# enoche/MMRec

Hardware: AMD Instinct MI355X
Metric: GCN-layer edges/sec (3-layer user-item CSR SpMM, d=64, fp32) (higher is better)
Workload: dtype f32

## Files before the change

### include/mmrec_hip.h

```cpp
#ifndef MMREC_HIP_H
#define MMREC_HIP_H

#include <stddef.h>
#include <stdint.h>

#ifdef __cplusplus
extern "C" {
#endif

#define MMREC_ABI_VERSION 16
#define MMREC_EMB_DIM 64

#define MMREC_ERR_BAD_ARG 10001
#define MMREC_ERR_UNSUPPORTED 10002

typedef void* mmrec_stream_t;

int mmrec_abi_version(void);
const char* mmrec_error_string(int err);

#ifndef MMREC_SPMM_CHUNK
#define MMREC_SPMM_CHUNK 512
#endif
#define MMREC_SPMM_LONG_ROW_DEFAULT 32
// ... 24 lines not shown
                             const float* Z, const float* acc_in, float* acc_out, int32_t n_rows, int32_t d, float alpha,
                             float beta, float acc_scale, int32_t long_row_threshold, const int32_t* long_rows,
                             const int32_t* long_chunk_ptr, int32_t n_long, int32_t n_chunks, float* partials,
                             int32_t* long_tickets, const int32_t* sched_row, const int32_t* sched_span,
                             const int32_t* sched_col, const float* sched_val, int32_t n_short, mmrec_stream_t stream);
int mmrec_spmm_csr_sched_f32_layergcn(const int32_t* rowptr, const int32_t* colidx, const float* vals, const float* X,
                                      float* Y, const float* ego, float* scaled, float* w, const float* acc_in,
                                      float* acc_out, int32_t n_rows, int32_t d, int32_t long_row_threshold,
                                      const int32_t* long_rows, const int32_t* long_chunk_ptr, int32_t n_long,
                                      int32_t n_chunks, float* partials, int32_t* long_tickets, const int32_t* sched_row,
                                      const int32_t* sched_span, const int32_t* sched_col, const float* sched_val,
                                      int32_t n_short, mmrec_stream_t stream);
int mmrec_spmm_row_keys(const int32_t* rowptr, const int32_t* colidx, const int32_t* col_degree, int32_t n_rows,
                        int32_t long_row_threshold, int32_t key_deg_max, int32_t* key, int32_t* key_degree,
                        mmrec_stream_t stream);

int mmrec_spmm_csr_masked_f32(const int32_t* rowptr, const int32_t* colidx, const float* vals, const float* X, float* Y,
                              const float* Z, const float* acc_in, float* acc_out, int32_t n_rows, int32_t d, float alpha,
                              float beta, float acc_scale, int32_t long_row_threshold, const int32_t* long_rows,
                              const int32_t* long_chunk_ptr, int32_t n_long, int32_t n_chunks, float* partials,
                              int32_t* long_tickets, const uint32_t* keep_bits, float val_scale, mmrec_stream_t stream);
int mmrec_edge_keep_bits(const uint8_t* keep, int64_t n_edges, const int64_t* perm_a, uint32_t* bits_a,
                         const int64_t* perm_b, uint32_t* bits_b, mmrec_stream_t stream);
int mmrec_spmm_plan_count(const int32_t* rowptr_host, int32_t n_rows, int32_t long_row_threshold,
                          int32_t* n_long, int32_t* n_chunks);
int mmrec_spmm_plan_fill(const int32_t* rowptr_host, int32_t n_rows, int32_t long_row_threshold,
                         int32_t* long_rows, int32_t* long_chunk_ptr);

int mmrec_cos_scale_fwd_f32(const float* E, const float* Ego, float* Out, float* w, float* acc,
                            int32_t n_rows, int32_t d, mmrec_stream_t stream);
int mmrec_cos_scale_bwd_f32(const float* dOut, const float* E, const float* Ego, const float* w,
                            float* dE, float* dEgo_accum, int32_t n_rows, int32_t d,
                            mmrec_stream_t stream);

#define MMREC_BPR_LOGSIG 0
#define MMREC_BPR_GAMMA 1

size_t mmrec_bpr_workspace_bytes(int32_t batch);
int mmrec_bpr_fwd_f32(const float* U, const float* P, const float* N, const int64_t* users,
                      const int64_t* pos, const int64_t* neg, int32_t batch, int32_t d,
                      int32_t variant, float scale, float* loss_out, float* coef, void* workspace,
                      mmrec_stream_t stream);
int mmrec_bpr_bwd_f32(const float* U, const float* P, const float* N, const int64_t* users,
                      const int64_t* pos, const int64_t* neg, int32_t batch, int32_t d,
                      const float* coef, const float* grad_scalar, float scale, float* dU, float* dP,
                      float* dN, mmrec_stream_t stream);
// ... 224 lines not shown
```

### mmrec_amd/_lib.py

```python
from __future__ import annotations

import ctypes
import os
from ctypes import c_char_p, c_float, c_int32, c_int64, c_size_t, c_uint64, c_void_p

import torch

_PKG = os.path.dirname(os.path.abspath(__file__))
LIB_PATH = os.environ.get("MMREC_HIP_LIB") or os.path.join(_PKG, "lib", "libmmrec_hip.so")
ABI_VERSION = 16

_P = c_void_p

SIGNATURES = {
    "mmrec_abi_version": (c_int32, []),
    "mmrec_error_string": (c_char_p, [c_int32]),
    "mmrec_spmm_csr_f32": (c_int32, [_P, _P, _P, _P, _P, _P, _P, _P, c_int32, c_int32, c_float,
                                     c_float, c_float, c_int32, _P, _P, c_int32, c_int32, _P, _P, _P]),
    "mmrec_spmm_csr_f32_layergcn": (c_int32, [_P, _P, _P, _P, _P, _P, _P, _P, _P, _P, c_int32, c_int32, c_int32,
                                              _P, _P, c_int32, c_int32, _P, _P, _P]),
    "mmrec_spmm_csr_sched_f32": (c_int32, [_P, _P, _P, _P, _P, _P, _P, _P, c_int32, c_int32, c_float,
                                           c_float, c_float, c_int32, _P, _P, c_int32, c_int32, _P, _P,
                                           _P, _P, _P, _P, c_int32, _P]),
    "mmrec_spmm_csr_sched_f32_layergcn": (c_int32, [_P, _P, _P, _P, _P, _P, _P, _P, _P, _P, c_int32, c_int32, c_int32,
                                                    _P, _P, c_int32, c_int32, _P, _P, _P, _P, _P, _P, c_int32, _P]),
    "mmrec_spmm_csr_masked_f32": (c_int32, [_P, _P, _P, _P, _P, _P, _P, _P, c_int32, c_int32, c_float,
                                            c_float, c_float, c_int32, _P, _P, c_int32, c_int32, _P, _P, _P, c_float, _P]),
    "mmrec_edge_keep_bits": (c_int32, [_P, c_int64, _P, _P, _P, _P, _P]),
    "mmrec_spmm_row_keys": (c_int32, [_P, _P, _P, c_int32, c_int32, c_int32, _P, _P, _P]),
    "mmrec_spmm_plan_count": (c_int32, [_P, c_int32, c_int32, _P, _P]),
    "mmrec_spmm_plan_fill": (c_int32, [_P, c_int32, c_int32, _P, _P]),
    "mmrec_cos_scale_fwd_f32": (c_int32, [_P, _P, _P, _P, _P, c_int32, c_int32, _P]),
    "mmrec_cos_scale_bwd_f32": (c_int32, [_P, _P, _P, _P, _P, _P, c_int32, c_int32, _P]),
    "mmrec_bpr_workspace_bytes": (c_size_t, [c_int32]),
    "mmrec_bpr_fwd_f32": (c_int32, [_P, _P, _P, _P, _P, _P, c_int32, c_int32, c_int32, c_float, _P,
                                    _P, _P, _P]),
    "mmrec_spmm_rows_f32": (c_int32, [_P, _P, _P, _P, _P, c_int32, _P, c_int32, c_int32, c_int32, _P, _P]),
    "mmrec_spmm_rows_any_f32": (c_int32, [_P, _P, _P, _P, _P, c_int32, _P, c_int32, c_int32, c_int32, c_int32, _P, _P]),
    "mmrec_spmm_push_rows_f32": (c_int32, [_P, _P, _P, _P, c_float, _P, c_int32, c_int32, _P, _P, _P]),
    "mmrec_bpr_dots_f32": (c_int32, [_P, _P, _P, _P, _P, _P, c_int32, c_int32, _P, _P]),
    "mmrec_bpr_loss_from_dots_f32": (c_int32, [_P, c_int32, c_int32, c_float, _P, _P, _P, _P]),
    "mmrec_bpr_bwd_f32": (c_int32, [_P, _P, _P, _P, _P, _P, c_int32, c_int32, _P, _P, c_float, _P, _P,
                                    _P, _P]),
    "mmrec_gather_sqnorm_fwd_f32": (c_int32, [_P, _P, c_int32, c_int32, _P, _P, _P]),
    "mmrec_gather_scale_add_bwd_f32": (c_int32, [_P, _P, c_int32, c_int32, _P, _P, _P]),
    "mmrec_infonce_workspace_bytes": (c_size_t, [c_int32]),
    "mmrec_infonce_fwd_f32": (c_int32, [_P, _P, _P, c_int32, c_int32, c_float, _P, _P, _P]),
    "mmrec_infonce_bwd_f32": (c_int32, [_P, c_int32, c_int32, c_float, _P, _P, _P, _P, _P]),
    "mmrec_linear_workspace_bytes": (c_size_t, [c_int32, c_int32, c_int32]),
    "mmrec_linear_fwd_f32": (c_int32, [_P, _P, _P, _P, c_int32, c_int32, c_int32, _P, _P]),
# ... 118 lines not shown
```

### mmrec_amd/csrc/spmm.hip

```cpp
#include "common.h"
#include "spmm_narrow.h"

#ifndef MMREC_SPMM_RPG
#define MMREC_SPMM_RPG(n_rows) ((n_rows) <= (1 << 18) ? 1 : 4)
#endif

namespace {

__device__ __forceinline__ void st_coherent(float4* p, float4 v) {
    unsigned long long* q = reinterpret_cast<unsigned long long*>(p);
    const unsigned long long lo = ((unsigned long long)__float_as_uint(v.y) << 32) | __float_as_uint(v.x);
    const unsigned long long hi = ((unsigned long long)__float_as_uint(v.w) << 32) | __float_as_uint(v.z);
    __hip_atomic_store(q, lo, __ATOMIC_RELAXED, __HIP_MEMORY_SCOPE_AGENT);
    __hip_atomic_store(q + 1, hi, __ATOMIC_RELAXED, __HIP_MEMORY_SCOPE_AGENT);
}
__device__ __forceinline__ float4 ld_coherent(const float4* p) {
    unsigned long long* q = reinterpret_cast<unsigned long long*>(const_cast<float4*>(p));
    const unsigned long long lo = __hip_atomic_load(q, __ATOMIC_RELAXED, __HIP_MEMORY_SCOPE_AGENT);
    const unsigned long long hi = __hip_atomic_load(q + 1, __ATOMIC_RELAXED, __HIP_MEMORY_SCOPE_AGENT);
    return make_float4(__uint_as_float((unsigned)lo), __uint_as_float((unsigned)(lo >> 32)),
                       __uint_as_float((unsigned)hi), __uint_as_float((unsigned)(hi >> 32)));
}

struct RowEpilogue {
    const float* Z;
    float* Y;
    const float* acc_in;
    float* acc_out;
    float alpha, beta, acc_scale;
    const float* ego;
    float* scaled;
    float* w_out;
};

struct RowSchedule {
    const int32_t* row;
    const int2* span;
    const int32_t* col;
    const float* val;
    int n_short;
};

template <int DCH, bool LG>
__device__ __forceinline__ void store_row(const RowEpilogue& ep, int row, int lane16, const float4 (&sum)[DCH]) {
    if (DCH == 1 && LG) {
        const size_t off = (size_t)row * 16 + lane16;
        const float4 y = f4_scale(ep.alpha, sum[0]);
        const float4 g = reinterpret_cast<const float4*>(ep.ego)[off];
        const float dot = row16_sum(f4_dot(y, g));
        const float ne = fmaxf(sqrtf(row16_sum(f4_dot(y, y))), 1e-8f);
        const float ng = fmaxf(sqrtf(row16_sum(f4_dot(g, g))), 1e-8f);
        const float w = dot / (ne * ng);
        const float4 o = f4_scale(w, y);
        if (ep.Y) reinterpret_cast<float4*>(ep.Y)[off] = y;
        reinterpret_cast<float4*>(ep.scaled)[off] = o;
        if (lane16 == 0) ep.w_out[row] = w;
        if (ep.acc_out)
            reinterpret_cast<float4*>(ep.acc_out)[off] =
                ep.acc_in ? f4_add(reinterpret_cast<const float4*>(ep.acc_in)[off], o) : o;
        return;
    }
#pragma unroll
    for (int ch = 0; ch < DCH; ++ch) {
        const size_t off = (size_t)row * (16 * DCH) + ch * 16 + lane16;
        float4 y = f4_scale(ep.alpha, sum[ch]);
        if (ep.Z) y = f4_fma(ep.beta, reinterpret_cast<const float4*>(ep.Z)[off], y);
        if (ep.Y) reinterpret_cast<float4*>(ep.Y)[off] = y;
// ... 19 lines not shown
            v = vals[k];
        }
        const int cnt = min(16, e - base);
        for (int j0 = 0; j0 < cnt; j0 += NB) {
            float4 x[NB][DCH];
            float vv[NB];
#pragma unroll
            for (int u = 0; u < NB; ++u) {
                const int j = j0 + u;
                const int cj = __shfl(c, j, 16);
                vv[u] = __shfl(v, j, 16);
#pragma unroll
                for (int ch = 0; ch < DCH; ++ch)
                    x[u][ch] = (j < cnt) ? X4[(size_t)cj * (16 * DCH) + ch * 16 + lane16] : f4_zero();
            }
#pragma unroll
            for (int u = 0; u < NB; ++u)
#pragma unroll
                for (int ch = 0; ch < DCH; ++ch) acc[ch] = f4_fma(vv[u], x[u][ch], acc[ch]);
        }
    }
}

template <int DCH, bool COHERENT, bool LG>
__device__ __forceinline__ void reduce_long_row(const float* __restrict__ partials, int c0, int c1, int row,
                                                const RowEpilogue& ep, float4 (*red)[16 * DCH]) {
    const int lane16 = threadIdx.x & 15, g = threadIdx.x >> 4;
#pragma unroll
    for (int ch = 0; ch < DCH; ++ch) {
        float4 t = f4_zero();
        for (int c = c0 + g; c < c1; c += 16) {
            const float4* src = reinterpret_cast<const float4*>(partials) + (size_t)c * (16 * DCH) + ch * 16 + lane16;
            t = f4_add(t, COHERENT ? ld_coherent(src) : *src);
        }
        red[g][ch * 16 + lane16] = t;
    }
    __syncthreads();
    if (g == 0) {
        float4 r[DCH];
#pragma unroll
        for (int ch = 0; ch < DCH; ++ch) {
            r[ch] = red[0][ch * 16 + lane16];
#pragma unroll
            for (int k = 1; k < 16; ++k) r[ch] = f4_add(r[ch], red[k][ch * 16 + lane16]);
        }
        store_row<DCH, LG>(ep, row, lane16, r);
    }
}

template <int DCH, bool LG, bool SCHED>
__global__ __launch_bounds__(256) void spmm_rows_kernel(
    const int32_t* __restrict__ rowptr, const int32_t* __restrict__ colidx,
    const float* __restrict__ vals, const float* __restrict__ X, RowEpilogue ep, int n_rows,
    int long_t, int rows_per_group, const int32_t* __restrict__ long_rows,
    const int32_t* __restrict__ long_chunk_ptr, int n_long, int n_chunks,
    float* __restrict__ partials, int32_t* __restrict__ tickets, RowSchedule sched) {
    __shared__ float4 red[16][16 * DCH];
    __shared__ int s_last;
    const int lane16 = threadIdx.x & 15;
    const int g = threadIdx.x >> 4;
    const float4* X4 = reinterpret_cast<const float4*>(X);
    if ((int)blockIdx.x < n_chunks) {
        const int chunk = blockIdx.x;
        int lo = 0, hi = n_long;
        while (hi - lo > 1) {
            const int mid = (lo + hi) >> 1;
            if (long_chunk_ptr[mid] <= chunk) lo = mid; else hi = mid;
        }
        const int row = long_rows[lo];
        const int cs = rowptr[row] + (chunk - long_chunk_ptr[lo]) * MMREC_SPMM_CHUNK;
        const int ce = min(cs + MMREC_SPMM_CHUNK, rowptr[row + 1]);
        float4 acc[DCH];
#pragma unroll
        for (int ch = 0; ch < DCH; ++ch) acc[ch] = f4_zero();
        for (int base = cs + g * 16; base < ce; base += 256)
            gather_span<DCH>(colidx, vals, X4, base, min(base + 16, ce), lane16, acc);
#pragma unroll
        for (int ch = 0; ch < DCH; ++ch) red[g][ch * 16 + lane16] = acc[ch];
        __syncthreads();
        if (g == 0) {
            float4 t[DCH];
#pragma unroll
            for (int ch = 0; ch < DCH; ++ch) {
                t[ch] = red[0][ch * 16 + lane16];
#pragma unroll
                for (int i = 1; i < 16; ++i) t[ch] = f4_add(t[ch], red[i][ch * 16 + lane16]);
            }
            if (long_chunk_ptr[lo + 1] - long_chunk_ptr[lo] == 1) {
                store_row<DCH, LG>(ep, row, lane16, t);
            } else {
#pragma unroll
                for (int ch = 0; ch < DCH; ++ch) {
                    float4* dst = reinterpret_cast<float4*>(partials) + (size_t)chunk * (16 * DCH) + ch * 16 + lane16;
                    if (tickets) st_coherent(dst, t[ch]); else *dst = t[ch];
                }
            }
        }
        const int c0 = long_chunk_ptr[lo], c1 = long_chunk_ptr[lo + 1];
        if (!tickets || c1 - c0 == 1) return;
        if (threadIdx.x < 64) {
            __atomic_signal_fence(__ATOMIC_SEQ_CST);
            __builtin_amdgcn_s_waitcnt(0);
            __atomic_signal_fence(__ATOMIC_SEQ_CST);
            __builtin_amdgcn_fence(__ATOMIC_RELEASE, "workgroup");
            if (threadIdx.x == 0)
                s_last = __hip_atomic_fetch_add(tickets + lo, 1, __ATOMIC_RELAXED, __HIP_MEMORY_SCOPE_AGENT) == c1 - c0 - 1;
        }
        __syncthreads();
        if (!s_last) return;
        __builtin_amdgcn_fence(__ATOMIC_ACQUIRE, "workgroup");
        reduce_long_row<DCH, true, LG>(partials, c0, c1, row, ep, red);
        if (threadIdx.x == 0) __hip_atomic_store(tickets + lo, 0, __ATOMIC_RELAXED, __HIP_MEMORY_SCOPE_AGENT);
        return;
    }
    if (SCHED) {
        const int slot0 = ((int)blockIdx.x - n_chunks) * 16 * rows_per_group + g;
#pragma unroll 1
        for (int i = 0; i < rows_per_group; ++i) {
            const int slot = slot0 + i * 16;
            if (slot >= sched.n_short) break;
            const int row = sched.row[slot];
            const int2 se = sched.span[slot];
            float4 acc[DCH];
#pragma unroll
            for (int ch = 0; ch < DCH; ++ch) acc[ch] = f4_zero();
            gather_span<DCH>(sched.col, sched.val, X4, se.x, se.y, lane16, acc);
            store_row<DCH, LG>(ep, row, lane16, acc);
        }
        return;
    }
    const int row0 = ((int)blockIdx.x - n_chunks) * 16 * rows_per_group + g;
#pragma unroll 1
    for (int i = 0; i < rows_per_group; ++i) {
        const int row = row0 + i * 16;
        if (row >= n_rows) break;
        const int s = rowptr[row], e = rowptr[row + 1];
        if (e - s > long_t) continue;
        float4 acc[DCH];
#pragma unroll
        for (int ch = 0; ch < DCH; ++ch) acc[ch] = f4_zero();
        gather_span<DCH>(colidx, vals, X4, s, e, lane16, acc);
        store_row<DCH, LG>(ep, row, lane16, acc);
    }
}

template <int DCH, bool LG>
__global__ __launch_bounds__(256) void spmm_long_reduce_kernel(
    const int32_t* __restrict__ long_rows, const int32_t* __restrict__ long_chunk_ptr, int n_long,
    const float* __restrict__ partials, RowEpilogue ep) {
    __shared__ float4 red[16][16 * DCH];
    const int i = blockIdx.x;
    const int c0 = long_chunk_ptr[i], c1 = long_chunk_ptr[i + 1];
    if (c1 - c0 <= 1) return;
    reduce_long_row<DCH, false, LG>(partials, c0, c1, long_rows[i], ep, red);
}

template <int DCH, bool LG = false, bool SCHED = false>
void launch_spmm(hipStream_t s, int blocks, int nch, const int32_t* rowptr, const int32_t* colidx,
                 const float* vals, const float* X, const RowEpilogue& ep, int n_rows, int long_t,
                 int rows_per_group, const int32_t* long_rows, const int32_t* long_chunk_ptr, int n_long,
                 float* partials, int32_t* tickets, const RowSchedule& sched = RowSchedule{}) {
    if (blocks + nch > 0)
        hipLaunchKernelGGL((spmm_rows_kernel<DCH, LG, SCHED>), dim3(blocks + nch), dim3(256), 0, s, rowptr, colidx, vals, X,
                           ep, n_rows, long_t, rows_per_group, long_rows, long_chunk_ptr, n_long, nch, partials, tickets,
                           sched);
    if (!tickets && n_long > 0 && nch > n_long)
        hipLaunchKernelGGL((spmm_long_reduce_kernel<DCH, LG>), dim3(n_long), dim3(256), 0, s, long_rows,
                           long_chunk_ptr, n_long, partials, ep);
}

template <int DCH>
__device__ __forceinline__ void gather_span_masked(const int32_t* __restrict__ colidx, const float* __restrict__ vals,
                                                   const uint32_t* __restrict__ keep_bits, float val_scale,
                                                   const float4* __restrict__ X4, int s, int e, int lane16,
                                                   float4 (&acc)[DCH]) {
    constexpr int NB = DCH == 1 ? 8 : (DCH <= 2 ? 4 : (DCH <= 4 ? 2 : 1));
    const int gshift = threadIdx.x & 48;
    for (int base = s; base < e; base += 16) {
        const int k = base + lane16;
        int c = 0;
        float v = 0.f;
        bool kept = false;
        if (k < e) {
            kept = (keep_bits[k >> 5] >> (k & 31)) & 1u;
            c = colidx[k];
            v = vals[k] * val_scale;
        }
        unsigned m = (unsigned)(__ballot(kept) >> gshift) & 0xffffu;
        while (m) {
            float4 x[NB][DCH];
            float vv[NB];
#pragma unroll
            for (int u = 0; u < NB; ++u) {
                const bool on = m != 0;
                const int j = on ? __ffs(m) - 1 : 0;
                m &= m - 1;
                const int cj = __shfl(c, j, 16);
                const float vj = __shfl(v, j, 16);
                vv[u] = on ? vj : 0.f;
#pragma unroll
                for (int ch = 0; ch < DCH; ++ch)
                    x[u][ch] = on ? X4[(size_t)cj * (16 * DCH) + ch * 16 + lane16] : f4_zero();
            }
#pragma unroll
            for (int u = 0; u < NB; ++u)
#pragma unroll
                for (int ch = 0; ch < DCH; ++ch) acc[ch] = f4_fma(vv[u], x[u][ch], acc[ch]);
        }
    }
}

template <int DCH>
__global__ __launch_bounds__(256) void spmm_rows_masked_kernel(
    const int32_t* __restrict__ rowptr, const int32_t* __restrict__ colidx, const float* __restrict__ vals,
    const uint32_t* __restrict__ keep_bits, float val_scale, const float* __restrict__ X, RowEpilogue ep, int n_rows,
    int long_t, int rows_per_group, const int32_t* __restrict__ long_rows, const int32_t* __restrict__ long_chunk_ptr,
    int n_long, int n_chunks, float* __restrict__ partials, int32_t* __restrict__ tickets) {
    __shared__ float4 red[16][16 * DCH];
    __shared__ int s_last;
    const int lane16 = threadIdx.x & 15;
    const int g = threadIdx.x >> 4;
    const float4* X4 = reinterpret_cast<const float4*>(X);
    if ((int)blockIdx.x < n_chunks) {
        const int chunk = blockIdx.x;
        int lo = 0, hi = n_long;
        while (hi - lo > 1) {
            const int mid = (lo + hi) >> 1;
            if (long_chunk_ptr[mid] <= chunk) lo = mid; else hi = mid;
        }
        const int row = long_rows[lo];
        const int cs = rowptr[row] + (chunk - long_chunk_ptr[lo]) * MMREC_SPMM_CHUNK;
        const int ce = min(cs + MMREC_SPMM_CHUNK, rowptr[row + 1]);
        float4 acc[DCH];
#pragma unroll
        for (int ch = 0; ch < DCH; ++ch) acc[ch] = f4_zero();
        for (int base = cs + g * 16; base < ce; base += 256)
            gather_span_masked<DCH>(colidx, vals, keep_bits, val_scale, X4, base, min(base + 16, ce), lane16, acc);
#pragma unroll
        for (int ch = 0; ch < DCH; ++ch) red[g][ch * 16 + lane16] = acc[ch];
        __syncthreads();
        const int c0 = long_chunk_ptr[lo], c1 = long_chunk_ptr[lo + 1];
        if (g == 0) {
            float4 t[DCH];
#pragma unroll
            for (int ch = 0; ch < DCH; ++ch) {
                t[ch] = red[0][ch * 16 + lane16];
#pragma unroll
                for (int i = 1; i < 16; ++i) t[ch] = f4_add(t[ch], red[i][ch * 16 + lane16]);
            }
            if (c1 - c0 == 1) {
                store_row<DCH, false>(ep, row, lane16, t);
            } else {
#pragma unroll
                for (int ch = 0; ch < DCH; ++ch) {
                    float4* dst = reinterpret_cast<float4*>(partials) + (size_t)chunk * (16 * DCH) + ch * 16 + lane16;
                    if (tickets) st_coherent(dst, t[ch]); else *dst = t[ch];
                }
            }
        }
        if (!tickets || c1 - c0 == 1) return;
        if (threadIdx.x < 64) {
            __atomic_signal_fence(__ATOMIC_SEQ_CST);
            __builtin_amdgcn_s_waitcnt(0);
            __atomic_signal_fence(__ATOMIC_SEQ_CST);
            __builtin_amdgcn_fence(__ATOMIC_RELEASE, "workgroup");
            if (threadIdx.x == 0)
                s_last = __hip_atomic_fetch_add(tickets + lo, 1, __ATOMIC_RELAXED, __HIP_MEMORY_SCOPE_AGENT) == c1 - c0 - 1;
        }
        __syncthreads();
        if (!s_last) return;
        __builtin_amdgcn_fence(__ATOMIC_ACQUIRE, "workgroup");
        reduce_long_row<DCH, true, false>(partials, c0, c1, row, ep, red);
        if (threadIdx.x == 0) __hip_atomic_store(tickets + lo, 0, __ATOMIC_RELAXED, __HIP_MEMORY_SCOPE_AGENT);
        return;
    }
    const int row0 = ((int)blockIdx.x - n_chunks) * 16 * rows_per_group + g;
#pragma unroll 1
    for (int i = 0; i < rows_per_group; ++i) {
        const int row = row0 + i * 16;
        if (row >= n_rows) break;
        const int s = rowptr[row], e = rowptr[row + 1];
        if (e - s > long_t) continue;
        float4 acc[DCH];
#pragma unroll
        for (int ch = 0; ch < DCH; ++ch) acc[ch] = f4_zero();
        gather_span_masked<DCH>(colidx, vals, keep_bits, val_scale, X4, s, e, lane16, acc);
        store_row<DCH, false>(ep, row, lane16, acc);
    }
}

template <int DCH>
void launch_spmm_masked(hipStream_t s, int blocks, int nch, const int32_t* rowptr, const int32_t* colidx, const float* vals,
                        const uint32_t* keep_bits, float val_scale, const float* X, const RowEpilogue& ep, int n_rows,
                        int long_t, int rows_per_group, const int32_t* long_rows, const int32_t* long_chunk_ptr, int n_long,
                        float* partials, int32_t* tickets) {
    if (blocks + nch > 0)
        hipLaunchKernelGGL((spmm_rows_masked_kernel<DCH>), dim3(blocks + nch), dim3(256), 0, s, rowptr, colidx, vals,
                           keep_bits, val_scale, X, ep, n_rows, long_t, rows_per_group, long_rows, long_chunk_ptr, n_long, nch,
                           partials, tickets);
    if (!tickets && n_long > 0 && nch > n_long)
        hipLaunchKernelGGL((spmm_long_reduce_kernel<DCH, false>), dim3(n_long), dim3(256), 0, s, long_rows,
                           long_chunk_ptr, n_long, partials, ep);
}

__global__ __launch_bounds__(256) void edge_keep_bits_kernel(const uint8_t* __restrict__ keep, long long n_edges,
                                                             const int64_t* __restrict__ perm_a,
                                                             uint32_t* __restrict__ bits_a,
                                                             const int64_t* __restrict__ perm_b,
                                                             uint32_t* __restrict__ bits_b) {
    const long long j = (long long)blockIdx.x * 256 + threadIdx.x;
    const long long n_words = (n_edges + 31) >> 5;
    const long long w = (j >> 6) * 2;
    const bool in = j < n_edges;
    const unsigned long long a = __ballot(in && keep[perm_a ? perm_a[j] : j] != 0);
    unsigned long long b = 0;
    if (bits_b) b = __ballot(in && keep[perm_b ? perm_b[j] : j] != 0);
    if ((threadIdx.x & 63) == 0 && w < n_words) {
        bits_a[w] = (uint32_t)a;
        if (w + 1 < n_words) bits_a[w + 1] = (uint32_t)(a >> 32);
        if (bits_b) {
            bits_b[w] = (uint32_t)b;
            if (w + 1 < n_words) bits_b[w + 1] = (uint32_t)(b >> 32);
        }
    }
// ... 282 lines not shown
                                                 float* partials, int32_t* long_tickets, const int32_t* sched_row,
                                                 const int32_t* sched_span, const int32_t* sched_col,
                                                 const float* sched_val, int32_t n_short, mmrec_stream_t stream) {
    if (d != MMREC_EMB_DIM) return MMREC_ERR_UNSUPPORTED;
    if (n_rows < 0 || n_long < 0 || n_chunks < 0 || long_row_threshold < 0) return MMREC_ERR_BAD_ARG;
    if (n_rows == 0) return 0;
    if (!rowptr || !X || !ego || !scaled || !w) return MMREC_ERR_BAD_ARG;
    if (n_long > 0 && (!long_rows || !long_chunk_ptr || !partials || n_chunks <= 0)) return MMREC_ERR_BAD_ARG;
    if (!sched_args_ok(sched_row, sched_span, sched_col, sched_val, n_short, n_rows)) return MMREC_ERR_BAD_ARG;
    if (Y == X || scaled == X || acc_out == X) return MMREC_ERR_BAD_ARG;
    RowEpilogue ep{nullptr, Y, acc_in, acc_out, 1.f, 0.f, 1.f, ego, scaled, w};
    const RowSchedule sched{sched_row, reinterpret_cast<const int2*>(sched_span), sched_col, sched_val, n_short};
    hipStream_t s = mmrec_stream(stream);
    const int rows_per_group = MMREC_SPMM_RPG(n_rows);
    const int blocks = (n_short + 16 * rows_per_group - 1) / (16 * rows_per_group);
    const int long_t = n_long > 0 ? long_row_threshold : INT32_MAX;
    const int nch = n_long > 0 ? n_chunks : 0;
    int32_t* tickets = n_long > 0 ? long_tickets : nullptr;
    launch_spmm<1, true, true>(s, blocks, nch, rowptr, colidx, vals, X, ep, n_rows, long_t, rows_per_group, long_rows,
                               long_chunk_ptr, n_long, partials, tickets, sched);
    MMREC_RETURN_LAUNCH_STATUS();
}

extern "C" int mmrec_spmm_row_keys(const int32_t* rowptr, const int32_t* colidx, const int32_t* col_degree,
                                   int32_t n_rows, int32_t long_row_threshold, int32_t key_deg_max, int32_t* key,
                                   int32_t* key_degree, mmrec_stream_t stream) {
    if (n_rows < 0 || long_row_threshold < 0 || key_deg_max < 0) return MMREC_ERR_BAD_ARG;
    if (n_rows == 0) return 0;
    if (!rowptr || !colidx || !col_degree || !key || !key_degree) return MMREC_ERR_BAD_ARG;
    hipLaunchKernelGGL(spmm_row_keys_kernel, dim3((n_rows + 15) / 16), dim3(256), 0, mmrec_stream(stream), rowptr, colidx,
                       col_degree, n_rows, long_row_threshold, key_deg_max, key, key_degree);
    MMREC_RETURN_LAUNCH_STATUS();
}

extern "C" int mmrec_spmm_plan_count(const int32_t* rowptr_host, int32_t n_rows,
                                     int32_t long_row_threshold, int32_t* n_long, int32_t* n_chunks) {
    if (!rowptr_host || !n_long || !n_chunks || n_rows < 0) return MMREC_ERR_BAD_ARG;
    int32_t nl = 0, nc = 0;
    for (int32_t r = 0; r < n_rows; ++r) {
        const int32_t deg = rowptr_host[r + 1] - rowptr_host[r];
        if (deg > long_row_threshold) {
            ++nl;
            nc += (deg + MMREC_SPMM_CHUNK - 1) / MMREC_SPMM_CHUNK;
        }
    }
    *n_long = nl;
// ... 44 lines not shown
```

### mmrec_amd/hip_ops.py

```python
from __future__ import annotations

import ctypes

import numpy as np
import torch

from . import _lib

EMB_DIM = 64
LINEAR_F16X3_DEFAULT = True
LINEAR_F16X3 = LINEAR_F16X3_DEFAULT
SLICE_WIDTHS = (8, 16, 32)
SPMM_CHUNK = 512
LONG_ROW_DEFAULT = None


def default_long_row_threshold(n_cols):
    import os
    forced = os.environ.get("MMREC_LONG_ROW_THRESHOLD")
    if forced:
        return int(forced)
    return 16 if n_cols <= (1 << 18) else 32


# ... 324 lines not shown
                                 (g.n_cols, tuple(X.shape)))
    for t, nm in ((Y, "Y"), (Z, "Z"), (acc_in, "acc_in"), (acc_out, "acc_out")):
        if t is not None:
            _chk(t, torch.float32, nm, 2)
            if t.shape[0] < g.n_rows or t.shape[1] != d:
                raise _lib.MMRecHipError("%s must be [>=%d, %d]" % (nm, g.n_rows, d))
    sc = g.scheduled(d)
    if sc is not None:
        g.checked(lib.mmrec_spmm_csr_sched_f32(_p(g.rowptr), _p(g.colidx), _p(g.vals), _p(X), _p(Y), _p(Z),
                                               _p(acc_in), _p(acc_out), g.n_rows, d, float(alpha),
                                               float(beta), float(acc_scale), g.long_row_threshold,
                                               _p(g.long_rows), _p(g.long_chunk_ptr), g.n_long, g.n_chunks,
                                               _p(g.partials_for(d)), _p(g.long_tickets), _p(sc["row"]), _p(sc["span"]),
                                               _p(sc["col"]), _p(sc["val"]), sc["n_short"], _stream()), "spmm_csr_sched_f32")
        return Y if Y is not None else acc_out
    g.checked(lib.mmrec_spmm_csr_f32(_p(g.rowptr), _p(g.colidx), _p(g.vals), _p(X), _p(Y), _p(Z),
                                     _p(acc_in), _p(acc_out), g.n_rows, d, float(alpha),
                                     float(beta), float(acc_scale), g.long_row_threshold,
                                     _p(g.long_rows), _p(g.long_chunk_ptr), g.n_long, g.n_chunks,
                                     _p(g.partials_for(d)), _p(g.long_tickets), _stream()), "spmm_csr_f32")
    return Y if Y is not None else acc_out


ROWS_MAX_CHUNKS = 480


def rows_servable(g: CsrGraph, d):
    if d not in SLICE_WIDTHS + (EMB_DIM,):
        return False
    return g.n_chunks == g.n_long or (d == EMB_DIM and g.max_row_chunks <= ROWS_MAX_CHUNKS)


def spmm_rows_raw(g: CsrGraph, X, rows, Z=None, z_compact=False):
    lib = _lib.load()
    _chk(X, torch.float32, "X", 2), _chk(rows, torch.int64, "rows", 1)
    d = X.shape[1]
    if not rows_servable(g, d) or X.shape[0] < g.n_cols:
        raise _lib.MMRecHipError("spmm_rows: graph with multi-chunk rows, or X not [>=%d, 8 / 16 / 32 / 64]" % g.n_cols)
    if Z is not None and (_chk(Z, torch.float32, "Z", 2).shape[0] < (rows.numel() if z_compact else g.n_rows) or Z.shape[1] != d):
        raise _lib.MMRecHipError("Z must be [>=%d, %d]" % (rows.numel() if z_compact else g.n_rows, d))
    Y = torch.empty(rows.numel(), d, dtype=torch.float32, device=X.device)
    long_t = g.long_row_threshold if g.n_long > 0 else 2 ** 31 - 1
    if g.n_chunks == g.n_long:
        _lib.check(lib.mmrec_spmm_rows_f32(_p(g.rowptr), _p(g.colidx), _p(g.vals), _p(X), _p(Z), 1 if z_compact else 0, _p(rows),
                                           rows.numel(), d, long_t, _p(Y), _stream()), "spmm_rows_f32")
    else:
# ... 64 lines not shown

def spmm(g: CsrGraph, X, Z=None):
    if isinstance(g, PermutedGraph):
        out = spmm(g.graph, g.to_new(X), None if Z is None else g.to_new(Z))
        return g.to_old(out)
    d = X.shape[1]
    if d % EMB_DIM and d not in SLICE_WIDTHS:
        pad = EMB_DIM - d % EMB_DIM
        Xp = torch.nn.functional.pad(X, (0, pad))
        Zp = None if Z is None else torch.nn.functional.pad(Z, (0, pad))
        return _SpMM.apply(Xp, Zp, g)[:, :d]
    return _SpMM.apply(X, Z, g)


class _LightGCNMean(torch.autograd.Function):

    @staticmethod
    def forward(ctx, E0, g, n_layers):
        ctx.g, ctx.L = g, int(n_layers)
        E0 = E0.contiguous()
        L = ctx.L
        if L == 0:
            return E0.clone()
        acc = torch.empty_like(E0)
        bufs = [torch.empty_like(E0) if L > 1 else None, torch.empty_like(E0) if L > 2 else None]
        cur = E0
        for layer in range(1, L + 1):
            last = layer == L
            Y = None if last else bufs[(layer - 1) % 2]
            spmm_raw(g, cur, Y=Y, acc_in=E0 if layer == 1 else acc, acc_out=acc,
                     acc_scale=1.0 / (L + 1) if last else 1.0)
            cur = Y
        return acc

    @staticmethod
    def backward(ctx, dOut):
        L, gt = ctx.L, ctx.g.transpose()
        dOut = dOut.contiguous()
        if L == 0:
            return dOut, None, None
        s = 1.0 / (L + 1)
        bufs = [torch.empty_like(dOut), torch.empty_like(dOut) if L > 1 else None]
        t = dOut
        for j in range(L):
            out = bufs[j % 2]
            spmm_raw(gt, t, Y=out, Z=dOut, alpha=s if j == 0 else 1.0, beta=s)
# ... 1196 lines not shown

def spmm_masked_raw(g: CsrGraph, vals, keep_bits, X, Y=None, Z=None, acc_in=None, acc_out=None, alpha=1.0, beta=1.0,
                    acc_scale=1.0, val_scale=1.0, tickets=True):
    lib = _lib.load()
    _chk(X, torch.float32, "X", 2), _chk(vals, torch.float32, "vals", 1), _chk(keep_bits, torch.int32, "keep_bits", 1)
    d = X.shape[1]
    if d % EMB_DIM or d > 6 * EMB_DIM or X.shape[0] < g.n_cols:
        raise _lib.MMRecHipError("X must be [>=%d, 64*k <= 384], got %s" % (g.n_cols, tuple(X.shape)))
    if vals.numel() != g.nnz or keep_bits.numel() * 32 < g.nnz:
        raise _lib.MMRecHipError("vals must be [%d] and keep_bits hold a bit for each" % g.nnz)
    for t, nm in ((Y, "Y"), (Z, "Z"), (acc_in, "acc_in"), (acc_out, "acc_out")):
        if t is not None:
            _chk(t, torch.float32, nm, 2)
            if t.shape[0] < g.n_rows or t.shape[1] != d:
                raise _lib.MMRecHipError("%s must be [>=%d, %d]" % (nm, g.n_rows, d))
    g.checked(lib.mmrec_spmm_csr_masked_f32(_p(g.rowptr), _p(g.colidx), _p(vals), _p(X), _p(Y), _p(Z), _p(acc_in),
                                            _p(acc_out), g.n_rows, d, float(alpha), float(beta), float(acc_scale),
                                            g.long_row_threshold, _p(g.long_rows), _p(g.long_chunk_ptr), g.n_long,
                                            g.n_chunks, _p(g.partials_for(d)), _p(g.long_tickets) if tickets else None,
                                            _p(keep_bits), float(val_scale), _stream()), "spmm_csr_masked_f32")
    return Y if Y is not None else acc_out


def _edge_dropout_values(eg, keep, scale):
    return (eg.vals * keep.to(eg.vals.dtype)) * scale


def _spmm_edge_dropout_composed(eg, X, keep, scale):
    return spmm_vals(eg.dyn, X, _edge_dropout_values(eg, keep, scale))


def _lightgcn_mean_edge_dropout_composed(eg, E0, n_layers, keep, scale):
    vals = _edge_dropout_values(eg, keep, scale)
    layers = [E0]
    for _ in range(int(n_layers)):
        E0 = spmm_vals(eg.dyn, E0, vals)
        layers.append(E0)
    return torch.stack(layers, dim=1).mean(dim=1)


class _SpMMEdgeDropout(torch.autograd.Function):
    @staticmethod
    def forward(ctx, X, eg, keep, scale):
        dyn = eg.dyn
        X = X.contiguous()
        bits_f, bits_b = edge_keep_bits(keep, dyn.perm, dyn.perm_t)
# ... 533 lines not shown
```

Before: 31.43 billion.

## Defer layer-mean accumulation into a final multi-addend SpMM epilogue

```diff
diff --git a/include/mmrec_hip.h b/include/mmrec_hip.h
--- a/include/mmrec_hip.h
+++ b/include/mmrec_hip.h
@@ -70,6 +70,24 @@
                               int32_t* long_tickets, const uint32_t* keep_bits, float val_scale, mmrec_stream_t stream);
 int mmrec_edge_keep_bits(const uint8_t* keep, int64_t n_edges, const int64_t* perm_a, uint32_t* bits_a,
                          const int64_t* perm_b, uint32_t* bits_b, mmrec_stream_t stream);
+int mmrec_spmm_csr_lsum_f32(const int32_t* rowptr, const int32_t* colidx, const float* vals, const float* X, float* Y,
+                            const float* Z, const float* add0, const float* add1, const float* add2, int32_t n_add,
+                            float* acc_out, int32_t n_rows, int32_t d, float alpha, float beta, float acc_scale,
+                            int32_t long_row_threshold, const int32_t* long_rows, const int32_t* long_chunk_ptr,
+                            int32_t n_long, int32_t n_chunks, float* partials, int32_t* long_tickets, mmrec_stream_t stream);
+int mmrec_spmm_csr_sched_lsum_f32(const int32_t* rowptr, const int32_t* colidx, const float* vals, const float* X, float* Y,
+                                  const float* Z, const float* add0, const float* add1, const float* add2, int32_t n_add,
+                                  float* acc_out, int32_t n_rows, int32_t d, float alpha, float beta, float acc_scale,
+                                  int32_t long_row_threshold, const int32_t* long_rows, const int32_t* long_chunk_ptr,
+                                  int32_t n_long, int32_t n_chunks, float* partials, int32_t* long_tickets,
+                                  const int32_t* sched_row, const int32_t* sched_span, const int32_t* sched_col,
+                                  const float* sched_val, int32_t n_short, mmrec_stream_t stream);
+int mmrec_spmm_csr_masked_lsum_f32(const int32_t* rowptr, const int32_t* colidx, const float* vals, const float* X, float* Y,
+                                   const float* Z, const float* add0, const float* add1, const float* add2, int32_t n_add,
+                                   float* acc_out, int32_t n_rows, int32_t d, float alpha, float beta, float acc_scale,
+                                   int32_t long_row_threshold, const int32_t* long_rows, const int32_t* long_chunk_ptr,
+                                   int32_t n_long, int32_t n_chunks, float* partials, int32_t* long_tickets,
+                                   const uint32_t* keep_bits, float val_scale, mmrec_stream_t stream);
 int mmrec_spmm_plan_count(const int32_t* rowptr_host, int32_t n_rows, int32_t long_row_threshold,
                           int32_t* n_long, int32_t* n_chunks);
 int mmrec_spmm_plan_fill(const int32_t* rowptr_host, int32_t n_rows, int32_t long_row_threshold,
diff --git a/mmrec_amd/_lib.py b/mmrec_amd/_lib.py
--- a/mmrec_amd/_lib.py
+++ b/mmrec_amd/_lib.py
@@ -26,6 +26,13 @@
                                                     _P, _P, c_int32, c_int32, _P, _P, _P, _P, _P, _P, c_int32, _P]),
     "mmrec_spmm_csr_masked_f32": (c_int32, [_P, _P, _P, _P, _P, _P, _P, _P, c_int32, c_int32, c_float,
                                             c_float, c_float, c_int32, _P, _P, c_int32, c_int32, _P, _P, _P, c_float, _P]),
+    "mmrec_spmm_csr_lsum_f32": (c_int32, [_P, _P, _P, _P, _P, _P, _P, _P, _P, c_int32, _P, c_int32, c_int32, c_float,
+                                          c_float, c_float, c_int32, _P, _P, c_int32, c_int32, _P, _P, _P]),
+    "mmrec_spmm_csr_sched_lsum_f32": (c_int32, [_P, _P, _P, _P, _P, _P, _P, _P, _P, c_int32, _P, c_int32, c_int32, c_float,
+                                                c_float, c_float, c_int32, _P, _P, c_int32, c_int32, _P, _P,
+                                                _P, _P, _P, _P, c_int32, _P]),
+    "mmrec_spmm_csr_masked_lsum_f32": (c_int32, [_P, _P, _P, _P, _P, _P, _P, _P, _P, c_int32, _P, c_int32, c_int32, c_float,
+                                                 c_float, c_float, c_int32, _P, _P, c_int32, c_int32, _P, _P, _P, c_float, _P]),
     "mmrec_edge_keep_bits": (c_int32, [_P, c_int64, _P, _P, _P, _P, _P]),
     "mmrec_spmm_row_keys": (c_int32, [_P, _P, _P, c_int32, c_int32, c_int32, _P, _P, _P]),
     "mmrec_spmm_plan_count": (c_int32, [_P, c_int32, c_int32, _P, _P]),
diff --git a/mmrec_amd/csrc/spmm.hip b/mmrec_amd/csrc/spmm.hip
--- a/mmrec_amd/csrc/spmm.hip
+++ b/mmrec_amd/csrc/spmm.hip
@@ -31,6 +31,9 @@
     const float* ego;
     float* scaled;
     float* w_out;
+    const float* add0;
+    const float* add1;
+    const float* add2;
 };
 
 struct RowSchedule {
@@ -41,8 +44,24 @@
     int n_short;
 };
 
-template <int DCH, bool LG>
+template <int DCH, bool LG, bool LS = false>
 __device__ __forceinline__ void store_row(const RowEpilogue& ep, int row, int lane16, const float4 (&sum)[DCH]) {
+    if (LS) {
+#pragma unroll
+        for (int ch = 0; ch < DCH; ++ch) {
+            const size_t off = (size_t)row * (16 * DCH) + ch * 16 + lane16;
+            float4 y = f4_scale(ep.alpha, sum[ch]);
+            if (ep.Z) y = f4_fma(ep.beta, reinterpret_cast<const float4*>(ep.Z)[off], y);
+            float4 a = reinterpret_cast<const float4*>(ep.add0)[off];
+            if (ep.add1) {
+                a = f4_add(a, reinterpret_cast<const float4*>(ep.add1)[off]);
+                if (ep.add2) a = f4_add(a, reinterpret_cast<const float4*>(ep.add2)[off]);
+            }
+            if (ep.Y) reinterpret_cast<float4*>(ep.Y)[off] = y;
+            reinterpret_cast<float4*>(ep.acc_out)[off] = f4_scale(ep.acc_scale, f4_add(a, y));
+        }
+        return;
+    }
     if (DCH == 1 && LG) {
         const size_t off = (size_t)row * 16 + lane16;
         const float4 y = f4_scale(ep.alpha, sum[0]);
@@ -108,7 +127,7 @@
     }
 }
 
-template <int DCH, bool COHERENT, bool LG>
+template <int DCH, bool COHERENT, bool LG, bool LS = false>
 __device__ __forceinline__ void reduce_long_row(const float* __restrict__ partials, int c0, int c1, int row,
                                                 const RowEpilogue& ep, float4 (*red)[16 * DCH]) {
     const int lane16 = threadIdx.x & 15, g = threadIdx.x >> 4;
@@ -130,11 +149,11 @@
 #pragma unroll
             for (int k = 1; k < 16; ++k) r[ch] = f4_add(r[ch], red[k][ch * 16 + lane16]);
         }
-        store_row<DCH, LG>(ep, row, lane16, r);
-    }
-}
-
-template <int DCH, bool LG, bool SCHED>
+        store_row<DCH, LG, LS>(ep, row, lane16, r);
+    }
+}
+
+template <int DCH, bool LG, bool SCHED, bool LS = false>
 __global__ __launch_bounds__(256) void spmm_rows_kernel(
     const int32_t* __restrict__ rowptr, const int32_t* __restrict__ colidx,
     const float* __restrict__ vals, const float* __restrict__ X, RowEpilogue ep, int n_rows,
@@ -173,7 +192,7 @@
                 for (int i = 1; i < 16; ++i) t[ch] = f4_add(t[ch], red[i][ch * 16 + lane16]);
             }
             if (long_chunk_ptr[lo + 1] - long_chunk_ptr[lo] == 1) {
-                store_row<DCH, LG>(ep, row, lane16, t);
+                store_row<DCH, LG, LS>(ep, row, lane16, t);
             } else {
 #pragma unroll
                 for (int ch = 0; ch < DCH; ++ch) {
@@ -195,7 +214,7 @@
         __syncthreads();
         if (!s_last) return;
         __builtin_amdgcn_fence(__ATOMIC_ACQUIRE, "workgroup");
-        reduce_long_row<DCH, true, LG>(partials, c0, c1, row, ep, red);
+        reduce_long_row<DCH, true, LG, LS>(partials, c0, c1, row, ep, red);
         if (threadIdx.x == 0) __hip_atomic_store(tickets + lo, 0, __ATOMIC_RELAXED, __HIP_MEMORY_SCOPE_AGENT);
         return;
     }
@@ -211,7 +230,7 @@
 #pragma unroll
             for (int ch = 0; ch < DCH; ++ch) acc[ch] = f4_zero();
             gather_span<DCH>(sched.col, sched.val, X4, se.x, se.y, lane16, acc);
-            store_row<DCH, LG>(ep, row, lane16, acc);
+            store_row<DCH, LG, LS>(ep, row, lane16, acc);
         }
         return;
     }
@@ -226,11 +245,11 @@
 #pragma unroll
         for (int ch = 0; ch < DCH; ++ch) acc[ch] = f4_zero();
         gather_span<DCH>(colidx, vals, X4, s, e, lane16, acc);
-        store_row<DCH, LG>(ep, row, lane16, acc);
-    }
-}
-
-template <int DCH, bool LG>
+        store_row<DCH, LG, LS>(ep, row, lane16, acc);
+    }
+}
+
+template <int DCH, bool LG, bool LS = false>
 __global__ __launch_bounds__(256) void spmm_long_reduce_kernel(
     const int32_t* __restrict__ long_rows, const int32_t* __restrict__ long_chunk_ptr, int n_long,
     const float* __restrict__ partials, RowEpilogue ep) {
@@ -238,20 +257,20 @@
     const int i = blockIdx.x;
     const int c0 = long_chunk_ptr[i], c1 = long_chunk_ptr[i + 1];
     if (c1 - c0 <= 1) return;
-    reduce_long_row<DCH, false, LG>(partials, c0, c1, long_rows[i], ep, red);
-}
-
-template <int DCH, bool LG = false, bool SCHED = false>
+    reduce_long_row<DCH, false, LG, LS>(partials, c0, c1, long_rows[i], ep, red);
+}
+
+template <int DCH, bool LG = false, bool SCHED = false, bool LS = false>
 void launch_spmm(hipStream_t s, int blocks, int nch, const int32_t* rowptr, const int32_t* colidx,
                  const float* vals, const float* X, const RowEpilogue& ep, int n_rows, int long_t,
                  int rows_per_group, const int32_t* long_rows, const int32_t* long_chunk_ptr, int n_long,
                  float* partials, int32_t* tickets, const RowSchedule& sched = RowSchedule{}) {
     if (blocks + nch > 0)
-        hipLaunchKernelGGL((spmm_rows_kernel<DCH, LG, SCHED>), dim3(blocks + nch), dim3(256), 0, s, rowptr, colidx, vals, X,
+        hipLaunchKernelGGL((spmm_rows_kernel<DCH, LG, SCHED, LS>), dim3(blocks + nch), dim3(256), 0, s, rowptr, colidx, vals, X,
                            ep, n_rows, long_t, rows_per_group, long_rows, long_chunk_ptr, n_long, nch, partials, tickets,
                            sched);
     if (!tickets && n_long > 0 && nch > n_long)
-        hipLaunchKernelGGL((spmm_long_reduce_kernel<DCH, LG>), dim3(n_long), dim3(256), 0, s, long_rows,
+        hipLaunchKernelGGL((spmm_long_reduce_kernel<DCH, LG, LS>), dim3(n_long), dim3(256), 0, s, long_rows,
                            long_chunk_ptr, n_long, partials, ep);
 }
 
@@ -296,7 +315,7 @@
     }
 }
 
-template <int DCH>
+template <int DCH, bool LS = false>
 __global__ __launch_bounds__(256) void spmm_rows_masked_kernel(
     const int32_t* __restrict__ rowptr, const int32_t* __restrict__ colidx, const float* __restrict__ vals,
     const uint32_t* __restrict__ keep_bits, float val_scale, const float* __restrict__ X, RowEpilogue ep, int n_rows,
@@ -335,7 +354,7 @@
                 for (int i = 1; i < 16; ++i) t[ch] = f4_add(t[ch], red[i][ch * 16 + lane16]);
             }
             if (c1 - c0 == 1) {
-                store_row<DCH, false>(ep, row, lane16, t);
+                store_row<DCH, false, LS>(ep, row, lane16, t);
             } else {
 #pragma unroll
                 for (int ch = 0; ch < DCH; ++ch) {
@@ -356,7 +375,7 @@
         __syncthreads();
         if (!s_last) return;
         __builtin_amdgcn_fence(__ATOMIC_ACQUIRE, "workgroup");
-        reduce_long_row<DCH, true, false>(partials, c0, c1, row, ep, red);
+        reduce_long_row<DCH, true, false, LS>(partials, c0, c1, row, ep, red);
         if (threadIdx.x == 0) __hip_atomic_store(tickets + lo, 0, __ATOMIC_RELAXED, __HIP_MEMORY_SCOPE_AGENT);
         return;
     }
@@ -371,21 +390,21 @@
 #pragma unroll
         for (int ch = 0; ch < DCH; ++ch) acc[ch] = f4_zero();
         gather_span_masked<DCH>(colidx, vals, keep_bits, val_scale, X4, s, e, lane16, acc);
-        store_row<DCH, false>(ep, row, lane16, acc);
-    }
-}
-
-template <int DCH>
+        store_row<DCH, false, LS>(ep, row, lane16, acc);
+    }
+}
+
+template <int DCH, bool LS = false>
 void launch_spmm_masked(hipStream_t s, int blocks, int nch, const int32_t* rowptr, const int32_t* colidx, const float* vals,
                         const uint32_t* keep_bits, float val_scale, const float* X, const RowEpilogue& ep, int n_rows,
                         int long_t, int rows_per_group, const int32_t* long_rows, const int32_t* long_chunk_ptr, int n_long,
                         float* partials, int32_t* tickets) {
     if (blocks + nch > 0)
-        hipLaunchKernelGGL((spmm_rows_masked_kernel<DCH>), dim3(blocks + nch), dim3(256), 0, s, rowptr, colidx, vals,
+        hipLaunchKernelGGL((spmm_rows_masked_kernel<DCH, LS>), dim3(blocks + nch), dim3(256), 0, s, rowptr, colidx, vals,
                            keep_bits, val_scale, X, ep, n_rows, long_t, rows_per_group, long_rows, long_chunk_ptr, n_long, nch,
                            partials, tickets);
     if (!tickets && n_long > 0 && nch > n_long)
-        hipLaunchKernelGGL((spmm_long_reduce_kernel<DCH, false>), dim3(n_long), dim3(256), 0, s, long_rows,
+        hipLaunchKernelGGL((spmm_long_reduce_kernel<DCH, false, LS>), dim3(n_long), dim3(256), 0, s, long_rows,
                            long_chunk_ptr, n_long, partials, ep);
 }
 
@@ -714,6 +733,119 @@
     MMREC_RETURN_LAUNCH_STATUS();
 }
 
+namespace {
+int lsum_args(const int32_t* rowptr, const float* X, const float* Y, const float* add0, const float* add1, const float* add2,
+              int32_t n_add, const float* acc_out, int32_t n_rows, int32_t d, int32_t long_row_threshold,
+              const int32_t* long_rows, const int32_t* long_chunk_ptr, int32_t n_long, int32_t n_chunks, const float* partials) {
+    if (d <= 0 || d % MMREC_EMB_DIM || d / MMREC_EMB_DIM > 6) return MMREC_ERR_UNSUPPORTED;
+    if (n_rows < 0 || n_long < 0 || n_chunks < 0 || long_row_threshold < 0) return MMREC_ERR_BAD_ARG;
+    if (n_add < 1 || n_add > 3) return MMREC_ERR_BAD_ARG;
+    if (n_rows == 0) return 0;
+    if (!rowptr || !X || !acc_out) return MMREC_ERR_BAD_ARG;
+    if (!add0 || (n_add > 1 && !add1) || (n_add > 2 && !add2)) return MMREC_ERR_BAD_ARG;
+    if (n_long > 0 && (!long_rows || !long_chunk_ptr || !partials || n_chunks <= 0)) return MMREC_ERR_BAD_ARG;
+    if (Y == X || acc_out == X) return MMREC_ERR_BAD_ARG;
+    return -1;
+}
+RowEpilogue lsum_epilogue(float* Y, const float* Z, const float* add0, const float* add1, const float* add2, int32_t n_add,
+                          float* acc_out, float alpha, float beta, float acc_scale) {
+    return RowEpilogue{Z, Y, nullptr, acc_out, alpha, Z ? beta : 0.f, acc_scale, nullptr, nullptr, nullptr,
+                       add0, n_add > 1 ? add1 : nullptr, n_add > 2 ? add2 : nullptr};
+}
+}
+
+#define MMREC_SPMM_DCH_SWITCH(d)                                                                                    \
+    switch ((d) / MMREC_EMB_DIM) {                                                                                  \
+        MMREC_SPMM_CASE(1) MMREC_SPMM_CASE(2) MMREC_SPMM_CASE(3) MMREC_SPMM_CASE(4) MMREC_SPMM_CASE(5)              \
+        MMREC_SPMM_CASE(6)                                                                                          \
+    }
+
+extern "C" int mmrec_spmm_csr_lsum_f32(const int32_t* rowptr, const int32_t* colidx, const float* vals, const float* X,
+                                       float* Y, const float* Z, const float* add0, const float* add1, const float* add2,
+                                       int32_t n_add, float* acc_out, int32_t n_rows, int32_t d, float alpha, float beta,
+                                       float acc_scale, int32_t long_row_threshold, const int32_t* long_rows,
+                                       const int32_t* long_chunk_ptr, int32_t n_long, int32_t n_chunks, float* partials,
+                                       int32_t* long_tickets, mmrec_stream_t stream) {
+    const int rc = lsum_args(rowptr, X, Y, add0, add1, add2, n_add, acc_out, n_rows, d, long_row_threshold, long_rows,
+                             long_chunk_ptr, n_long, n_chunks, partials);
+    if (rc >= 0) return rc;
+    const RowEpilogue ep = lsum_epilogue(Y, Z, add0, add1, add2, n_add, acc_out, alpha, beta, acc_scale);
+    hipStream_t s = mmrec_stream(stream);
+    const int rows_per_group = MMREC_SPMM_RPG(n_rows);
+    const int blocks = (n_rows + 16 * rows_per_group - 1) / (16 * rows_per_group);
+    const int long_t = n_long > 0 ? long_row_threshold : INT32_MAX;
+    const int nch = n_long > 0 ? n_chunks : 0;
+    int32_t* tickets = n_long > 0 ? long_tickets : nullptr;
+#define MMREC_SPMM_CASE(D)                                                                                          \
+    case D:                                                                                                         \
+        launch_spmm<D, false, false, true>(s, blocks, nch, rowptr, colidx, vals, X, ep, n_rows, long_t,             \
+                                           rows_per_group, long_rows, long_chunk_ptr, n_long, partials, tickets);   \
+        break;
+    MMREC_SPMM_DCH_SWITCH(d)
+#undef MMREC_SPMM_CASE
+    MMREC_RETURN_LAUNCH_STATUS();
+}
+
+extern "C" int mmrec_spmm_csr_sched_lsum_f32(const int32_t* rowptr, const int32_t* colidx, const float* vals, const float* X,
+                                             float* Y, const float* Z, const float* add0, const float* add1,
+                                             const float* add2, int32_t n_add, float* acc_out, int32_t n_rows, int32_t d,
+                                             float alpha, float beta, float acc_scale, int32_t long_row_threshold,
+                                             const int32_t* long_rows, const int32_t* long_chunk_ptr, int32_t n_long,
+                                             int32_t n_chunks, float* partials, int32_t* long_tickets,
+                                             const int32_t* sched_row, const int32_t* sched_span, const int32_t* sched_col,
+                                             const float* sched_val, int32_t n_short, mmrec_stream_t stream) {
+    const int rc = lsum_args(rowptr, X, Y, add0, add1, add2, n_add, acc_out, n_rows, d, long_row_threshold, long_rows,
+                             long_chunk_ptr, n_long, n_chunks, partials);
+    if (rc >= 0) return rc;
+    if (!sched_args_ok(sched_row, sched_span, sched_col, sched_val, n_short, n_rows)) return MMREC_ERR_BAD_ARG;
+    const RowEpilogue ep = lsum_epilogue(Y, Z, add0, add1, add2, n_add, acc_out, alpha, beta, acc_scale);
+    const RowSchedule sched{sched_row, reinterpret_cast<const int2*>(sched_span), sched_col, sched_val, n_short};
+    hipStream_t s = mmrec_stream(stream);
+    const int rows_per_group = MMREC_SPMM_RPG(n_rows);
+    const int blocks = (n_short + 16 * rows_per_group - 1) / (16 * rows_per_group);
+    const int long_t = n_long > 0 ? long_row_threshold : INT32_MAX;
+    const int nch = n_long > 0 ? n_chunks : 0;
+    int32_t* tickets = n_long > 0 ? long_tickets : nullptr;
+#define MMREC_SPMM_CASE(D)                                                                                          \
+    case D:                                                                                                         \
+        launch_spmm<D, false, true, true>(s, blocks, nch, rowptr, colidx, vals, X, ep, n_rows, long_t,              \
+                                          rows_per_group, long_rows, long_chunk_ptr, n_long, partials, tickets,     \
+                                          sched);                                                                   \
+        break;
+    MMREC_SPMM_DCH_SWITCH(d)
+#undef MMREC_SPMM_CASE
+    MMREC_RETURN_LAUNCH_STATUS();
+}
+
+extern "C" int mmrec_spmm_csr_masked_lsum_f32(const int32_t* rowptr, const int32_t* colidx, const float* vals, const float* X,
+                                              float* Y, const float* Z, const float* add0, const float* add1,
+                                              const float* add2, int32_t n_add, float* acc_out, int32_t n_rows, int32_t d,
+                                              float alpha, float beta, float acc_scale, int32_t long_row_threshold,
+                                              const int32_t* long_rows, const int32_t* long_chunk_ptr, int32_t n_long,
+                                              int32_t n_chunks, float* partials, int32_t* long_tickets,
+                                              const uint32_t* keep_bits, float val_scale, mmrec_stream_t stream) {
+    const int rc = lsum_args(rowptr, X, Y, add0, add1, add2, n_add, acc_out, n_rows, d, long_row_threshold, long_rows,
+                             long_chunk_ptr, n_long, n_chunks, partials);
+    if (rc >= 0) return rc;
+    if (!keep_bits) return MMREC_ERR_BAD_ARG;
+    const RowEpilogue ep = lsum_epilogue(Y, Z, add0, add1, add2, n_add, acc_out, alpha, beta, acc_scale);
+    hipStream_t s = mmrec_stream(stream);
+    const int rows_per_group = MMREC_SPMM_RPG(n_rows);
+    const int blocks = (n_rows + 16 * rows_per_group - 1) / (16 * rows_per_group);
+    const int long_t = n_long > 0 ? long_row_threshold : INT32_MAX;
+    const int nch = n_long > 0 ? n_chunks : 0;
+    int32_t* tickets = n_long > 0 ? long_tickets : nullptr;
+#define MMREC_SPMM_CASE(D)                                                                                          \
+    case D:                                                                                                         \
+        launch_spmm_masked<D, true>(s, blocks, nch, rowptr, colidx, vals, keep_bits, val_scale, X, ep, n_rows,      \
+                                    long_t, rows_per_group, long_rows, long_chunk_ptr, n_long, partials, tickets);  \
+        break;
+    MMREC_SPMM_DCH_SWITCH(d)
+#undef MMREC_SPMM_CASE
+    MMREC_RETURN_LAUNCH_STATUS();
+}
+#undef MMREC_SPMM_DCH_SWITCH
+
 extern "C" int mmrec_spmm_row_keys(const int32_t* rowptr, const int32_t* colidx, const int32_t* col_degree,
                                    int32_t n_rows, int32_t long_row_threshold, int32_t key_deg_max, int32_t* key,
                                    int32_t* key_degree, mmrec_stream_t stream) {
diff --git a/mmrec_amd/hip_ops.py b/mmrec_amd/hip_ops.py
--- a/mmrec_amd/hip_ops.py
+++ b/mmrec_amd/hip_ops.py
@@ -370,6 +370,63 @@
     return Y if Y is not None else acc_out
 
 
+def _lsum_check(g, X, addends, acc_out, Y, Z, what):
+    _chk(X, torch.float32, "X", 2)
+    d = X.shape[1]
+    if d % EMB_DIM or d > 6 * EMB_DIM or X.shape[0] < g.n_cols:
+        raise _lib.MMRecHipError("%s: X must be [>=%d, 64*k <= 384], got %s" % (what, g.n_cols, tuple(X.shape)))
+    addends = list(addends)
+    if not 1 <= len(addends) <= 3:
+        raise _lib.MMRecHipError("%s: 1 to 3 addend tables, got %d" % (what, len(addends)))
+    if acc_out is None:
+        raise _lib.MMRecHipError("%s: acc_out is required" % what)
+    for t, nm in [(Y, "Y"), (Z, "Z"), (acc_out, "acc_out")] + [(a, "addend %d" % i) for i, a in enumerate(addends)]:
+        if t is not None or nm.startswith("addend"):
+            _chk(t, torch.float32, nm, 2)
+            if t.shape[0] < g.n_rows or t.shape[1] != d:
+                raise _lib.MMRecHipError("%s must be [>=%d, %d]" % (nm, g.n_rows, d))
+    return d, [_p(a) for a in addends] + [None] * (3 - len(addends)), len(addends)
+
+
+def spmm_lsum_raw(g: CsrGraph, X, addends, acc_out, Y=None, Z=None, alpha=1.0, beta=1.0, acc_scale=1.0, tickets=True):
+    lib = _lib.load()
+    d, (a0, a1, a2), n_add = _lsum_check(g, X, addends, acc_out, Y, Z, "spmm_lsum")
+    tk = _p(g.long_tickets) if tickets else None
+    sc = g.scheduled(d)
+    if sc is not None:
+        g.checked(lib.mmrec_spmm_csr_sched_lsum_f32(_p(g.rowptr), _p(g.colidx), _p(g.vals), _p(X), _p(Y), _p(Z), a0, a1, a2,
+                                                    n_add, _p(acc_out), g.n_rows, d, float(alpha), float(beta),
+                                                    float(acc_scale), g.long_row_threshold, _p(g.long_rows),
+                                                    _p(g.long_chunk_ptr), g.n_long, g.n_chunks, _p(g.partials_for(d)), tk,
+                                                    _p(sc["row"]), _p(sc["span"]), _p(sc["col"]), _p(sc["val"]), sc["n_short"],
+                                                    _stream()), "spmm_csr_sched_lsum_f32")
+        return acc_out
+    g.checked(lib.mmrec_spmm_csr_lsum_f32(_p(g.rowptr), _p(g.colidx), _p(g.vals), _p(X), _p(Y), _p(Z), a0, a1, a2, n_add,
+                                          _p(acc_out), g.n_rows, d, float(alpha), float(beta), float(acc_scale),
+                                          g.long_row_threshold, _p(g.long_rows), _p(g.long_chunk_ptr), g.n_long, g.n_chunks,
+                                          _p(g.partials_for(d)), tk, _stream()), "spmm_csr_lsum_f32")
+    return acc_out
+
+
+def _layer_mean_launches(E0, L, plain, lsum):
+    out = torch.empty_like(E0)
+    bufs = [torch.empty_like(E0), torch.empty_like(E0) if L > 2 else None]
+    pending, cur = [E0], E0
+    for layer in range(1, L + 1):
+        if layer == L:
+            lsum(cur, None, pending, out, 1.0 / (L + 1))
+            break
+        Y = bufs[(layer - 1) % 2]
+        if L >= 4 and layer % 2 == 0:
+            lsum(cur, Y, pending, out, 1.0)
+            pending = [out]
+        else:
+            plain(cur, Y)
+            pending.append(Y)
+        cur = Y
+    return out
+
+
 ROWS_MAX_CHUNKS = 480
 
 
@@ -480,6 +537,10 @@
         L = ctx.L
         if L == 0:
             return E0.clone()
+        if L >= 2 and E0.shape[1] % EMB_DIM == 0:
+            return _layer_mean_launches(
+                E0, L, lambda X, Y: spmm_raw(g, X, Y=Y),
+                lambda X, Y, adds, out, sc: spmm_lsum_raw(g, X, adds, out, Y=Y, acc_scale=sc))
         acc = torch.empty_like(E0)
         bufs = [torch.empty_like(E0) if L > 1 else None, torch.empty_like(E0) if L > 2 else None]
         cur = E0
@@ -1722,6 +1783,21 @@
     return Y if Y is not None else acc_out
 
 
+def spmm_masked_lsum_raw(g: CsrGraph, vals, keep_bits, X, addends, acc_out, Y=None, Z=None, alpha=1.0, beta=1.0,
+                         acc_scale=1.0, val_scale=1.0, tickets=True):
+    lib = _lib.load()
+    _chk(vals, torch.float32, "vals", 1), _chk(keep_bits, torch.int32, "keep_bits", 1)
+    d, (a0, a1, a2), n_add = _lsum_check(g, X, addends, acc_out, Y, Z, "spmm_masked_lsum")
+    if vals.numel() != g.nnz or keep_bits.numel() * 32 < g.nnz:
+        raise _lib.MMRecHipError("vals must be [%d] and keep_bits hold a bit for each" % g.nnz)
+    g.checked(lib.mmrec_spmm_csr_masked_lsum_f32(_p(g.rowptr), _p(g.colidx), _p(vals), _p(X), _p(Y), _p(Z), a0, a1, a2, n_add,
+                                                 _p(acc_out), g.n_rows, d, float(alpha), float(beta), float(acc_scale),
+                                                 g.long_row_threshold, _p(g.long_rows), _p(g.long_chunk_ptr), g.n_long,
+                                                 g.n_chunks, _p(g.partials_for(d)), _p(g.long_tickets) if tickets else None,
+                                                 _p(keep_bits), float(val_scale), _stream()), "spmm_csr_masked_lsum_f32")
+    return acc_out
+
+
 def _edge_dropout_values(eg, keep, scale):
     return (eg.vals * keep.to(eg.vals.dtype)) * scale
 
```

Result: no change. 31.15 billion (-0.9%).
